# Minys233/GCN-BMP

Measured on AMD Instinct MI355X. Metric: drug-pairs/sec fwd+bwd, binary-DDI GGNN d=128, higher is better.
Workload: dtype f32; 1 GPU; C2: full binary DDI set (544 drugs, 147696 pairs), GGNN 4-step d=128 tied + Nie co-attention (head 8, tanh) + MLP(32,16), fwd+bwd+Adam, 1024 pairs/GPU/step, every molecule instance encoded; the 144 batches of one epoch resident in HBM, cycled; layout=per-instance packed layout, whole 128-row tiles, pairs_per_gpu=1024, global_batch=1024, parallelism=dp1

## Files before the change

gcn-bmp_amd/csrc/bmp_fused.hip:

```cpp
#include <type_traits>
#include <string.h>
#include "bmp_kernels.h"

#include "bmp_tile.h"

template <int D, bool FIRST, bool VAR, bool SAVE>
__global__ __launch_bounds__(512) void k_ggnn_step_fwd(StepArgs a) {
    constexpr int LD = D + 4;
    constexpr int NCB = D / 32, NRW = 8 / NCB, RB = 4 / NRW;
    extern __shared__ __attribute__((aligned(16))) float lds[];
    float* Hs = lds;
    float* As = lds + FZ_R * LD;
    float* wds = As + FZ_R * LD;
    int* rptr = (int*)(wds + FZ_R * 4);
    int* ecol = rptr + 132;
    float* evalv = (float*)(ecol + FZ_ECAP);
    int* sy = (int*)(evalv + FZ_ECAP);

    const int tid = threadIdx.x, lane = tid & 63, w = tid >> 6;
    const int grp = w >> 2;
    GrpSync gs{sy + grp, 0};
    if (tid < FZ_NSYNC) sy[tid] = 0;
    if (grp == 0) __builtin_amdgcn_s_setprio(2);
    const int wc = w % NCB, wr = w / NCB;
    const int l31 = lane & 31, hi = lane >> 5;
    FZ_TILE_SETUP();
    if (VAR && a.tile_stride > nrows) {
        const int e = row0 + a.tile_stride;
        fz_clear_rows<512>(a.hout, D, row0 + nrows, e, tid);
        fz_clear_rows<512>(a.m, D, row0 + nrows, e, tid);
        fz_clear_rows<512>(a.rz, 2 * D, row0 + nrows, e, tid);
        fz_clear_rows<512>(a.c, D, row0 + nrows, e, tid);
    }
    const int col = wc * 32 + l31;
    const int wrow0 = wr * RB * 32;
    const int lrow = wrow0 + 4 * hi;
    const int rot = (tile * 8) % D;
    const float* Hw = Hs + (wrow0 + l31) * LD + 4 * hi;
    const float* Aw = As + (wrow0 + l31) * LD + 4 * hi;
    float* Hl = Hs + lrow * LD + col;
    float* Al = As + lrow * LD + col;
#define LOFF(rb, reg) (((rb) * 32 + ((reg) & 3) + 8 * ((reg) >> 2)) * LD)

    constexpr bool save = SAVE;
    for (int idx = tid; idx < nrows * (D / 4); idx += 512) {
        const int r = idx / (D / 4), c4 = idx % (D / 4);
        *(f32x4*)(Hs + r * LD + 4 * c4) = *(const f32x4*)(a.h + (size_t)(row0 + r) * D + 4 * c4);
    }
    const bool csr_lds = stage_csr(a.ptr, a.col, a.val, row0, rptr, ecol, evalv, nrows);
    __syncthreads();
    if (!grp_live) return;
    const RowOrder ro = FZ_ROW_ORDER();
    const int bi = wr & 1;

    auto step = [&](auto first_c, const float* WTs, const float* bEs, const float* ATs, const float* bvs, float* om, float* orz,
                    float* oc, float* oh) {
        constexpr bool FST = decltype(first_c)::value;
        int tmask = 0;
        f32x16 acc_m[1][RB];
        zero_acc(acc_m[0]);
        for (int e = 0; e < 4; ++e) {
            const float* const Bp[1] = {WTs + (size_t)(e * D + 4 * hi) * D + 4 * col};
            const int ldw[1] = {D};
            BPre<1> pre;
            tile_b_prefetch<1>(pre, Bp, ldw, D, rot);
            float wd;
            FZ_GATHER(Hs, As, e, &wd);
            if ((tid & 3) == 0) wds[(tid >> 2) * 4 + e] = wd;
            if (e == 0 && (tid & 3) == 0 && tmask) __hip_atomic_fetch_or(sy + 2 + grp, tmask, __ATOMIC_RELAXED, __HIP_MEMORY_SCOPE_WORKGROUP);
            grp_sync(gs);
            const int any = (__hip_atomic_load(sy + 2 + grp, __ATOMIC_RELAXED, __HIP_MEMORY_SCOPE_WORKGROUP) >> e) & 1;
            if (any) tile_mma_msg<VAR, 1, RB>(nrb, e, ro.nbr, bi, acc_m, Aw, LD, Bp, ldw, D, rot, &pre);
            FZ_GSYNC();
        }
        constexpr int NG = FST ? 2 : 3;
        int ldwg[NG];
    #pragma unroll
        for (int g = 0; g < NG; ++g) ldwg[g] = 3 * D;
        const float* const base_h = ATs + (size_t)(4 * hi) * 3 * D + 4 * col + (FST ? 4 * D : 0);
        const float* const base_m = ATs + (size_t)(D + 4 * hi) * 3 * D + 4 * col + (FST ? 4 * D : 0);
        const float* Bh[NG]; const float* Bm[NG];
    #pragma unroll
        for (int g = 0; g < NG; ++g) { Bh[g] = base_h + 4 * D * g; Bm[g] = base_m + 4 * D * g; }
        BPre<NG> pre_h;
        tile_b_prefetch<NG>(pre_h, (const float* const (&)[NG])Bh, (const int (&)[NG])ldwg, D, rot);
        {
            const AccBuf mo = acc_buf<D>(om, row0, 0, col);
            float be[4];
    #pragma unroll
            for (int e = 0; e < 4; ++e) be[e] = bEs[e * D + col];
            FZ_FOR_ACC {
                const int tp = lrow + rb * 32 + (reg & 3) + 8 * (reg >> 2);
                const int r = (tp & 64) + ro.perm[tp];
                const f32x4 wd4 = *(const f32x4*)(wds + r * 4);
                const float v = __builtin_fmaf(wd4[3], be[3], __builtin_fmaf(wd4[2], be[2], __builtin_fmaf(wd4[1], be[1],
                                               __builtin_fmaf(wd4[0], be[0], acc_m[0][rb][reg]))));
                As[r * LD + col] = v;
                if (save) __builtin_amdgcn_raw_buffer_store_b32(__builtin_bit_cast(unsigned, v), mo.rs, mo.vo + r * D * 4, 0, 0);
            }
        }
        FZ_GSYNC();

        f32x16 acc_g[3][RB];
        zero_acc(acc_g[0]); zero_acc(acc_g[1]); zero_acc(acc_g[2]);
        {
            f32x16 gg[NG][RB];
    #pragma unroll
            for (int g = 0; g < NG; ++g) zero_acc(gg[g]);
            BPre<NG> pre_m;
            tile_b_prefetch<NG>(pre_m, (const float* const (&)[NG])Bm, (const int (&)[NG])ldwg, D, rot);
            tile_mma_n<VAR, NG, RB>(nrb, gg, Hw, LD, (const float* const (&)[NG])Bh, (const int (&)[NG])ldwg, D, rot, &pre_h);
            tile_mma_n<VAR, NG, RB>(nrb, gg, Aw, LD, (const float* const (&)[NG])Bm, (const int (&)[NG])ldwg, D, rot, &pre_m);
    #pragma unroll
            for (int g = 0; g < NG; ++g)
    #pragma unroll
                for (int rb = 0; rb < RB; ++rb) acc_g[g + (FST ? 1 : 0)][rb] = gg[g][rb];
        }
        const float br = bvs[col], bz = bvs[D + col], bcn = bvs[2 * D + col];
        {
            const AccBuf rzo = acc_buf<2 * D>(orz, row0, lrow, col);
            FZ_FOR_ACC {
                const float zv = bmp_sigmoid(acc_g[1][rb][reg] + bz);
                acc_g[1][rb][reg] = zv;
                if (save) acc_st<2 * D>(rzo, rb, reg, zv, D);
                if (!FST) {
                    const float rv = bmp_sigmoid(acc_g[0][rb][reg] + br);
                    acc_g[0][rb][reg] = rv;
                    if (save) acc_st<2 * D>(rzo, rb, reg, rv, 0);
                }
            }
        }
        if (!FST) {
            const float* const Bu[1] = {a.UcT + (size_t)(4 * hi) * D + 4 * col};
            const int ldu[1] = {D};
            BPre<1> pre_u;
            tile_b_prefetch<1>(pre_u, Bu, ldu, D, rot);
            FZ_GSYNC();
            FZ_FOR_ACC { Al[LOFF(rb, reg)] = acc_g[0][rb][reg] * Hl[LOFF(rb, reg)]; }
            FZ_GSYNC();
            f32x16 gc[1][RB];
    #pragma unroll
            for (int rb = 0; rb < RB; ++rb) gc[0][rb] = acc_g[2][rb];
            tile_mma_n<VAR, 1, RB>(nrb, gc, Aw, LD, Bu, ldu, D, rot, &pre_u);
    #pragma unroll
            for (int rb = 0; rb < RB; ++rb) acc_g[2][rb] = gc[0][rb];
        }
        {
            const AccBuf co = acc_buf<D>(oc, row0, lrow, col);
            const AccBuf ho = acc_buf<D>(oh, row0, lrow, col);
            FZ_FOR_ACC {
                const float cv = bmp_tanh(acc_g[2][rb][reg] + bcn);
                const float zv = acc_g[1][rb][reg];
                float hn = zv * cv;
                if (!FST) hn = __builtin_fmaf(1.f - zv, Hl[LOFF(rb, reg)], hn);
                if (save) acc_st<D>(co, rb, reg, cv);
                acc_st<D>(ho, rb, reg, hn);
            }
        }
    };
    step(std::integral_constant<bool, FIRST>{}, a.WT, a.bE, a.AT, a.b, a.m, a.rz, a.c, a.hout);
}

template <int D, bool FIRST, bool VAR>
__global__ __launch_bounds__(512) void k_ggnn_step_bwd(StepArgs a) {
    constexpr int LD = D + 4;
    constexpr int NCB = D / 32, NRW = 8 / NCB, RB = 4 / NRW;
    constexpr int F4 = D / 4;
    constexpr int NV = D / 16;
    extern __shared__ __attribute__((aligned(16))) float lds[];
    float* Xs = lds;
    float* Ys = lds + FZ_R * LD;
    int* rptr = (int*)(Ys + FZ_R * LD + FZ_R * 4);
    int* ecol = rptr + 132;
    float* evalv = (float*)(ecol + FZ_ECAP);
    int* sy = (int*)(evalv + FZ_ECAP);

    const int tid = threadIdx.x, lane = tid & 63, w = tid >> 6;
    const int grp = w >> 2;
    GrpSync gs{sy + grp, 0};
    int tmask = 0;
    if (tid < FZ_NSYNC) sy[tid] = 0;
    if (grp == 0) __builtin_amdgcn_s_setprio(2);
    const int wc = w % NCB, wr = w / NCB;
    const int l31 = lane & 31, hi = lane >> 5;
    FZ_TILE_SETUP();
    if (VAR && a.tile_stride > nrows) {
        const int e = row0 + a.tile_stride;
        fz_clear_rows<512>(a.dh, D, row0 + nrows, e, tid);
        fz_clear_rows<512>(a.gda, 7 * D, row0 + nrows, e, tid);
    }
    const int col = wc * 32 + l31;
    const int wrow0 = wr * RB * 32;
    const int lrow = wrow0 + 4 * hi;
    const int rot = (tile * 8) % D;
    const float* Xw = Xs + (wrow0 + l31) * LD + 4 * hi;
    const float* Yw = Ys + (wrow0 + l31) * LD + 4 * hi;
    float* Xl = Xs + lrow * LD + col;
    float* Yl = Ys + lrow * LD + col;
    constexpr bool first = FIRST;
    const int tg = tid & 255;
#define RM_ROW(v) (grp * 64 + ((v) * 256 + tg) / F4)
#define RM_C4(v) (((v) * 256 + tg) % F4)
#define RM_LDS(T, v) (*(f32x4*)((T) + RM_ROW(v) * LD + 4 * RM_C4(v)))
#define RM_LIVE(v) (!VAR || grp * 64 + (v) * (256 / F4) < nrows)
    const AccBuf b_g = rm_buf<D, D>(a.dhout, row0, grp, tg), b_c = rm_buf<D, D>(a.c, row0, grp, tg);
    const AccBuf b_h = rm_buf<D, D>(a.h, row0, grp, tg), b_rz = rm_buf<D, 2 * D>(a.rz, row0, grp, tg);
    const AccBuf b_o = rm_buf<D, 7 * D>(a.gda, row0, grp, tg), b_dh = rm_buf<D, D>(a.dh, row0, grp, tg);

    const bool csr_lds = stage_csr(a.ptr, a.col, a.val, row0, rptr, ecol, evalv, nrows);
    if (!grp_live) {
        __syncthreads();
        return;
    }

    f32x4 ex[NV];
    {
        const f32x4 one = (f32x4){1.f, 1.f, 1.f, 1.f};
        f32x4 g4[NV], z4[NV], c4[NV], h4[NV];
#pragma unroll
        for (int v = 0; v < NV; ++v) if (RM_LIVE(v)) {
            g4[v] = rm_ld<D, D>(b_g, v);
            z4[v] = rm_ld<D, 2 * D>(b_rz, v, D);
            c4[v] = rm_ld<D, D>(b_c, v);
            if (!first) h4[v] = rm_ld<D, D>(b_h, v);
        }
#pragma unroll
        for (int v = 0; v < NV; ++v) if (RM_LIVE(v)) {
            const f32x4 gz = g4[v] * z4[v];
            const f32x4 dac = gz * (one - c4[v] * c4[v]);
            f32x4 dz = gz * (one - z4[v]);
            if (first) { dz *= c4[v]; ex[v] = (f32x4){0.f, 0.f, 0.f, 0.f}; }
            else { dz *= (c4[v] - h4[v]); ex[v] = g4[v] - gz; }
            RM_LDS(Xs, v) = dac;
            RM_LDS(Ys, v) = dz;
            rm_st<D, 7 * D>(b_o, v, dac, 6 * D);
            rm_st<D, 7 * D>(b_o, v, dz, 5 * D);
        }
    }
    const float* const Ac_h = a.A + (size_t)(2 * D + 4 * hi) * 2 * D + 4 * col;
    const float* const Az_h = a.A + (size_t)(D + 4 * hi) * 2 * D + 4 * col;
    const float* const Ar_h = a.A + (size_t)(4 * hi) * 2 * D + 4 * col;
    const int ld2[2] = {2 * D, 2 * D};
    const float* const Bc[2] = {Ac_h, Ac_h + 4 * D};
    BPre<2> pre_c;
    tile_b_prefetch<2>(pre_c, Bc, ld2, D, rot);
    __syncthreads();
    const RowOrder ro = FZ_ROW_ORDER();
    const int bi = wr & 1;
    int aoff[RB];
#pragma unroll
    for (int rb = 0; rb < RB; ++rb) { const int tp = wrow0 + rb * 32 + l31; aoff[rb] = (((tp & 64) + ro.perm[tp]) - (wrow0 + l31)) * LD; }
#define FZ_ROWOF(rb, reg) ((lrow & 64) + ro.perm[lrow + (rb) * 32 + ((reg) & 3) + 8 * ((reg) >> 2)])

    f32x16 acc_x[2][RB];
    zero_acc(acc_x[0]); zero_acc(acc_x[1]);
    tile_mma_n<VAR, 2, RB>(nrb, acc_x, Xw, LD, Bc, ld2, D, rot, &pre_c, aoff);
    if (!first) {
        f32x16 acc_d[1][RB];
        zero_acc(acc_d[0]);
        {
            const float* const Bu[1] = {a.Uc + (size_t)(4 * hi) * D + 4 * col};
            const int ldu[1] = {D};
            tile_mma_n<VAR, 1, RB>(nrb, acc_d, Xw, LD, Bu, ldu, D, rot, nullptr, aoff);
        }
        FZ_GSYNC();
        FZ_FOR_ACC { Xs[FZ_ROWOF(rb, reg) * LD + col] = acc_d[0][rb][reg]; }
        f32x4 r4[NV], h4[NV];
#pragma unroll
        for (int v = 0; v < NV; ++v) if (RM_LIVE(v)) { r4[v] = rm_ld<D, 2 * D>(b_rz, v); h4[v] = rm_ld<D, D>(b_h, v); }
        FZ_GSYNC();
#pragma unroll
        for (int v = 0; v < NV; ++v) if (RM_LIVE(v)) {
            const f32x4 drh = RM_LDS(Xs, v);
            const f32x4 dr = drh * r4[v];
            const f32x4 dar = dr * h4[v] * ((f32x4){1.f, 1.f, 1.f, 1.f} - r4[v]);
            ex[v] += dr;
            RM_LDS(Xs, v) = dar;
            rm_st<D, 7 * D>(b_o, v, dar, 4 * D);
        }
        FZ_GSYNC();
        {
            const float* const Br[2] = {Ar_h, Ar_h + 4 * D};
            tile_mma_n<VAR, 2, RB>(nrb, acc_x, Xw, LD, Br, ld2, D, rot, nullptr, aoff);
        }
    }
    {
        const float* const Bz[2] = {Az_h, Az_h + 4 * D};
        tile_mma_n<VAR, 2, RB>(nrb, acc_x, Yw, LD, Bz, ld2, D, rot, nullptr, aoff);
    }
    FZ_GSYNC();
    FZ_FOR_ACC { Xs[FZ_ROWOF(rb, reg) * LD + col] = acc_x[1][rb][reg]; }
    __syncthreads();

    f32x16 acc_h[1][RB];
#pragma unroll
    for (int rb = 0; rb < RB; ++rb) acc_h[0][rb] = acc_x[0][rb];
    for (int e = 0; e < 4; ++e) {
        const float* const Bp[1] = {a.Wnat + (size_t)(4 * hi) * 4 * D + 4 * (e * D + col)};
        const int ldw[1] = {4 * D};
        BPre<1> pre;
        tile_b_prefetch<1>(pre, Bp, ldw, D, rot);
        float wd;
        const bool has_e = FZ_GATHER(Xs, Ys, e, &wd);
        if ((tid >> 2) < nrows && (has_e || !a.skip_zero_g)) {
            const int row = tid >> 2, q = tid & 3;
            const float* s = Ys + ((row & 64) + ro.inv[row]) * LD + q * (D / 4);
            float* o = a.gda + (size_t)(row0 + row) * 7 * D + e * D + q * (D / 4);
#pragma unroll
            for (int f = 0; f < D / 16; ++f) *(f32x4*)(o + 4 * f) = *(const f32x4*)(s + 4 * f);
        }
        if (e == 0 && (tid & 3) == 0 && tmask) __hip_atomic_fetch_or(sy + 2 + grp, tmask, __ATOMIC_RELAXED, __HIP_MEMORY_SCOPE_WORKGROUP);
        grp_sync(gs);
        const int any = (__hip_atomic_load(sy + 2 + grp, __ATOMIC_RELAXED, __HIP_MEMORY_SCOPE_WORKGROUP) >> e) & 1;
        if (any) tile_mma_msg<VAR, 1, RB>(nrb, e, ro.nbr, bi, acc_h, Yw, LD, Bp, ldw, D, rot, &pre);
        FZ_GSYNC();
    }
    FZ_FOR_ACC { Ys[FZ_ROWOF(rb, reg) * LD + col] = acc_h[0][rb][reg]; }
    FZ_GSYNC();
#pragma unroll
    for (int v = 0; v < NV; ++v) if (RM_LIVE(v)) rm_st<D, D>(b_dh, v, RM_LDS(Ys, v) + ex[v]);
#undef RM_LIVE
#undef RM_ROW
#undef RM_C4
#undef RM_LDS
#undef FZ_ROWOF
}

struct RelArgs {
    const int* ptr; const int* col; const float* val;
    int tile0;
    int act;
    const int* mt_row0; const int* mt_nblk;
    int mt_rows;
    const float* h;
    const float* WT;
    const float* bE;
    const float* WsT;
    const float* bs;
    float* out;
    float* wdeg;
    const float* dout; const float* y;
    const float* Wnat;
    const float* Ws;
    float* dh;
    float* gda;
    int skip_zero_g;
};

template <int D, bool VAR>
__global__ __launch_bounds__(512) void k_relgcn_layer_fwd(RelArgs a) {
    constexpr int LD = D + 4;
    constexpr int NCB = D / 32, NRW = 8 / NCB, RB = 4 / NRW;
    extern __shared__ __attribute__((aligned(16))) float lds[];
    float* Hs = lds;
    float* As = lds + FZ_R * LD;
    float* wds = As + FZ_R * LD;
    int* rptr = (int*)(wds + FZ_R * 4);
    int* ecol = rptr + 132;
    float* evalv = (float*)(ecol + FZ_ECAP);
    int* sy = (int*)(evalv + FZ_ECAP);

    const int tid = threadIdx.x, lane = tid & 63, w = tid >> 6;
    const int grp = w >> 2;
    GrpSync gs{sy + grp, 0};
    int tmask = 0;
    if (tid < FZ_NSYNC) sy[tid] = 0;
    if (grp == 0) __builtin_amdgcn_s_setprio(2);
    const int wc = w % NCB, wr = w / NCB;
    const int l31 = lane & 31, hi = lane >> 5;
    FZ_TILE_SETUP();
    const int col = wc * 32 + l31;
    const int wrow0 = wr * RB * 32;
    const int lrow = wrow0 + 4 * hi;
    const int rot = (tile * 8) % D;
    const float* Hw = Hs + (wrow0 + l31) * LD + 4 * hi;
    const float* Aw = As + (wrow0 + l31) * LD + 4 * hi;

    for (int idx = tid; idx < nrows * (D / 4); idx += 512) {
        const int r = idx / (D / 4), c4 = idx % (D / 4);
        *(f32x4*)(Hs + r * LD + 4 * c4) = *(const f32x4*)(a.h + (size_t)(row0 + r) * D + 4 * c4);
    }
    const bool csr_lds = stage_csr(a.ptr, a.col, a.val, row0, rptr, ecol, evalv, nrows);
    __syncthreads();
    if (!grp_live) return;
    const RowOrder ro = FZ_ROW_ORDER();
    const int bi = wr & 1;
    int aoff[RB];
#pragma unroll
    for (int rb = 0; rb < RB; ++rb) { const int tp = wrow0 + rb * 32 + l31; aoff[rb] = (((tp & 64) + ro.perm[tp]) - (wrow0 + l31)) * LD; }

    f32x16 acc[1][RB];
    zero_acc(acc[0]);
    const float* const Bs[1] = {a.WsT + (size_t)(4 * hi) * D + 4 * col};
    const int lds_[1] = {D};
    BPre<1> pre_s;
    for (int e = 0; e < 4; ++e) {
        const float* const Bp[1] = {a.WT + (size_t)(e * D + 4 * hi) * D + 4 * col};
        const int ldw[1] = {D};
        BPre<1> pre;
        tile_b_prefetch<1>(pre, Bp, ldw, D, rot);
        if (e == 3) tile_b_prefetch<1>(pre_s, Bs, lds_, D, rot);
        float wd;
        FZ_GATHER(Hs, As, e, &wd);
        if ((tid & 3) == 0) wds[(tid >> 2) * 4 + e] = wd;
        if (e == 0 && (tid & 3) == 0 && tmask) __hip_atomic_fetch_or(sy + 2 + grp, tmask, __ATOMIC_RELAXED, __HIP_MEMORY_SCOPE_WORKGROUP);
        grp_sync(gs);
        const int any = (__hip_atomic_load(sy + 2 + grp, __ATOMIC_RELAXED, __HIP_MEMORY_SCOPE_WORKGROUP) >> e) & 1;
        if (any) tile_mma_msg<VAR, 1, RB>(nrb, e, ro.nbr, bi, acc, Aw, LD, Bp, ldw, D, rot, &pre);
        FZ_GSYNC();
    }
    tile_mma_n<VAR, 1, RB>(nrb, acc, Hw, LD, Bs, lds_, D, rot, &pre_s, aoff);
    {
        const AccBuf oo = acc_buf<D>(a.out, row0, 0, col);
        float be[4];
#pragma unroll
        for (int e = 0; e < 4; ++e) be[e] = a.bE[e * D + col];
        const float bsv = a.bs ? a.bs[col] : 0.f;
        const int act = a.act;
        FZ_FOR_ACC {
            const int tp = lrow + rb * 32 + (reg & 3) + 8 * (reg >> 2);
            const int r = (tp & 64) + ro.perm[tp];
            const f32x4 wd4 = *(const f32x4*)(wds + r * 4);
            const float v = acc[0][rb][reg] + bsv + wd4[0] * be[0] + wd4[1] * be[1] + wd4[2] * be[2] + wd4[3] * be[3];
            __builtin_amdgcn_raw_buffer_store_b32(__builtin_bit_cast(unsigned, bmp_act(act, v)), oo.rs, oo.vo + r * D * 4, 0, 0);
        }
    }
    if (a.wdeg != nullptr && (tid & 255) < 64 && grp * 64 + (tid & 255) < nrows) {
        const int r = grp * 64 + (tid & 255);
        *(f32x4*)(a.wdeg + (size_t)(row0 + r) * 4) = *(const f32x4*)(wds + r * 4);
    }
}

template <int D, bool VAR>
__global__ __launch_bounds__(512) void k_relgcn_layer_bwd(RelArgs a) {
    constexpr int LD = D + 4;
    constexpr int NCB = D / 32, NRW = 8 / NCB, RB = 4 / NRW;
    constexpr int F4 = D / 4;
    constexpr int NV = D / 16;
    extern __shared__ __attribute__((aligned(16))) float lds[];
    float* Xs = lds;
    float* Ys = lds + FZ_R * LD;
    int* rptr = (int*)(Ys + FZ_R * LD + FZ_R * 4);
    int* ecol = rptr + 132;
    float* evalv = (float*)(ecol + FZ_ECAP);
    int* sy = (int*)(evalv + FZ_ECAP);

    const int tid = threadIdx.x, lane = tid & 63, w = tid >> 6;
    const int grp = w >> 2;
    GrpSync gs{sy + grp, 0};
    int tmask = 0;
    if (tid < FZ_NSYNC) sy[tid] = 0;
    if (grp == 0) __builtin_amdgcn_s_setprio(2);
    const int wc = w % NCB, wr = w / NCB;
    const int l31 = lane & 31, hi = lane >> 5;
    FZ_TILE_SETUP();
    const int col = wc * 32 + l31;
    const int wrow0 = wr * RB * 32;
    const int lrow = wrow0 + 4 * hi;
    const int rot = (tile * 8) % D;
    const float* Xw = Xs + (wrow0 + l31) * LD + 4 * hi;
    const float* Yw = Ys + (wrow0 + l31) * LD + 4 * hi;
    float* Yl = Ys + lrow * LD + col;
    const int tg = tid & 255;
#define RM_ROW(v) (grp * 64 + ((v) * 256 + tg) / F4)
#define RM_C4(v) (((v) * 256 + tg) % F4)
#define RM_LDS(T, v) (*(f32x4*)((T) + RM_ROW(v) * LD + 4 * RM_C4(v)))
#define RM_LIVE(v) (!VAR || grp * 64 + (v) * (256 / F4) < nrows)
    const AccBuf b_g = rm_buf<D, D>(a.dout, row0, grp, tg), b_y = rm_buf<D, D>(a.y, row0, grp, tg);
    const AccBuf b_o = rm_buf<D, 5 * D>(a.gda, row0, grp, tg), b_dh = rm_buf<D, D>(a.dh, row0, grp, tg);

    const bool csr_lds = stage_csr(a.ptr, a.col, a.val, row0, rptr, ecol, evalv, nrows);
    if (!grp_live) {
        __syncthreads();
        return;
    }

    {
        f32x4 g4[NV], y4[NV];
#pragma unroll
        for (int v = 0; v < NV; ++v) if (RM_LIVE(v)) { g4[v] = rm_ld<D, D>(b_g, v); y4[v] = rm_ld<D, D>(b_y, v); }
        const int act = a.act;
#pragma unroll
        for (int v = 0; v < NV; ++v) if (RM_LIVE(v)) {
            f32x4 dp;
#pragma unroll
            for (int t = 0; t < 4; ++t) dp[t] = g4[v][t] * bmp_dact(act, y4[v][t]);
            RM_LDS(Xs, v) = dp;
            rm_st<D, 5 * D>(b_o, v, dp, 4 * D);
        }
    }
    const float* const Bs[1] = {a.Ws + (size_t)(4 * hi) * D + 4 * col};
    const int lds_[1] = {D};
    BPre<1> pre_s;
    tile_b_prefetch<1>(pre_s, Bs, lds_, D, rot);
    __syncthreads();
    const RowOrder ro = FZ_ROW_ORDER();
    const int bi = wr & 1;
    int aoff[RB];
#pragma unroll
    for (int rb = 0; rb < RB; ++rb) { const int tp = wrow0 + rb * 32 + l31; aoff[rb] = (((tp & 64) + ro.perm[tp]) - (wrow0 + l31)) * LD; }

    f32x16 acc_h[1][RB];
    zero_acc(acc_h[0]);
    tile_mma_n<VAR, 1, RB>(nrb, acc_h, Xw, LD, Bs, lds_, D, rot, &pre_s, aoff);
    for (int e = 0; e < 4; ++e) {
        const float* const Bp[1] = {a.Wnat + (size_t)(4 * hi) * 4 * D + 4 * (e * D + col)};
        const int ldw[1] = {4 * D};
        BPre<1> pre;
        tile_b_prefetch<1>(pre, Bp, ldw, D, rot);
        float wd;
        const bool has_e = FZ_GATHER(Xs, Ys, e, &wd);
        if ((tid >> 2) < nrows && (has_e || !a.skip_zero_g)) {
            const int row = tid >> 2, q = tid & 3;
            const float* s = Ys + ((row & 64) + ro.inv[row]) * LD + q * (D / 4);
            float* o = a.gda + (size_t)(row0 + row) * 5 * D + e * D + q * (D / 4);
#pragma unroll
            for (int f = 0; f < D / 16; ++f) *(f32x4*)(o + 4 * f) = *(const f32x4*)(s + 4 * f);
        }
        if (e == 0 && (tid & 3) == 0 && tmask) __hip_atomic_fetch_or(sy + 2 + grp, tmask, __ATOMIC_RELAXED, __HIP_MEMORY_SCOPE_WORKGROUP);
        grp_sync(gs);
        const int any = (__hip_atomic_load(sy + 2 + grp, __ATOMIC_RELAXED, __HIP_MEMORY_SCOPE_WORKGROUP) >> e) & 1;
        if (any) tile_mma_msg<VAR, 1, RB>(nrb, e, ro.nbr, bi, acc_h, Yw, LD, Bp, ldw, D, rot, &pre);
        FZ_GSYNC();
    }
    FZ_FOR_ACC {
        const int tp = lrow + rb * 32 + (reg & 3) + 8 * (reg >> 2);
        Ys[((tp & 64) + ro.perm[tp]) * LD + col] = acc_h[0][rb][reg];
    }
    FZ_GSYNC();
#pragma unroll
    for (int v = 0; v < NV; ++v) if (RM_LIVE(v)) rm_st<D, D>(b_dh, v, RM_LDS(Ys, v));
#undef RM_LIVE
#undef RM_ROW
#undef RM_C4
#undef RM_LDS
}

struct ROArgs {
    const float* h; const float* h0;
    const float* WT;
    const float* b;
    int act_j;
    const float* row_w; const int* row_mol; const int* mol_nrows;
    float* ij;
    float* g;
};

template <int D, bool HAS0>
__global__ __launch_bounds__(512) void k_readout_tile_fwd(ROArgs a) {
    constexpr int LD = D + 4;
    constexpr int NCB = D / 32, NRW = 8 / NCB, RB = 4 / NRW;
    extern __shared__ __attribute__((aligned(16))) float lds[];
    float* Hs = lds;
    float* As = lds + FZ_R * LD;
    int* mlist = (int*)(As + FZ_R * LD);
    float* rws = (float*)(mlist + 400);
    const int tid = threadIdx.x, lane = tid & 63, w = tid >> 6;
    const int wc = w % NCB, wr = w / NCB;
    const int l31 = lane & 31, hi = lane >> 5;
    const int row0 = blockIdx.x * FZ_R;
    const int col = wc * 32 + l31;
    const int wrow0 = wr * RB * 32;
    const int lrow = wrow0 + 4 * hi;
    const int rot = (blockIdx.x * 8) % D;
    constexpr int nrb = RB;
    const float* Hw = Hs + (wrow0 + l31) * LD + 4 * hi;
    const float* Aw = As + (wrow0 + l31) * LD + 4 * hi;
    float* Al = As + lrow * LD + col;

    for (int idx = tid; idx < FZ_R * (D / 4); idx += 512) {
        const int r = idx / (D / 4), c4 = idx % (D / 4);
        *(f32x4*)(Hs + r * LD + 4 * c4) = *(const f32x4*)(a.h + (size_t)(row0 + r) * D + 4 * c4);
        if (HAS0) *(f32x4*)(As + r * LD + 4 * c4) = *(const f32x4*)(a.h0 + (size_t)(row0 + r) * D + 4 * c4);
    }
    if (tid < FZ_R) rws[tid] = a.row_w[row0 + tid];
    const float* const Bh[2] = {a.WT + (size_t)(4 * hi) * 2 * D + 4 * col, a.WT + (size_t)(4 * hi) * 2 * D + 4 * (D + col)};
    const int ldw[2] = {2 * D, 2 * D};
    BPre<2> pre_h;
    tile_b_prefetch<2>(pre_h, Bh, ldw, D, rot);
    __syncthreads();

    f32x16 acc[2][RB];
    zero_acc(acc[0]); zero_acc(acc[1]);
    if (HAS0) {
        const float* const B0[2] = {Bh[0] + (size_t)D * 2 * D, Bh[1] + (size_t)D * 2 * D};
        BPre<2> pre_0;
        tile_b_prefetch<2>(pre_0, B0, ldw, D, rot);
        tile_mma<2, RB>(acc, Hw, LD, Bh, ldw, D, rot, &pre_h);
        tile_mma<2, RB>(acc, Aw, LD, B0, ldw, D, rot, &pre_0);
    } else {
        tile_mma<2, RB>(acc, Hw, LD, Bh, ldw, D, rot, &pre_h);
    }
    if (tid < FZ_R) {
        const int mol = a.row_mol[row0 + tid];
        const int prev = tid > 0 ? a.row_mol[row0 + tid - 1] : -2;
        const bool head = mol >= 0 && mol != prev;
        const unsigned long long bal = __ballot(head);
        if (lane == 0) mlist[128 + w] = __popcll(bal);
        const int before = __popcll(bal & ((1ull << lane) - 1ull));
        if (head) { mlist[130 + tid] = before; }
        mlist[260 + tid] = head ? mol : -1;
    }
    __syncthreads();
    {
        const AccBuf io = acc_buf<2 * D>(a.ij, row0, lrow, col);
        const float bi = a.b ? a.b[col] : 0.f, bj = a.b ? a.b[D + col] : 0.f;
        const int act = a.act_j;
        FZ_FOR_ACC {
            const int r = lrow + rb * 32 + (reg & 3) + 8 * (reg >> 2);
            const float iv = bmp_sigmoid(acc[0][rb][reg] + bi);
            const float jv = bmp_act(act, acc[1][rb][reg] + bj);
            if (a.ij != nullptr) {
                acc_st<2 * D>(io, rb, reg, iv, 0);
                acc_st<2 * D>(io, rb, reg, jv, D);
            }
            Al[LOFF(rb, reg)] = rws[r] * iv * jv;
        }
    }
    if (tid < FZ_R && mlist[260 + tid] >= 0) {
        const int idx = mlist[130 + tid] + (tid >= 64 ? mlist[128] : 0);
        mlist[2 * idx] = tid;
        mlist[2 * idx + 1] = mlist[260 + tid];
    }
// ... 255 lines not shown
```

gcn-bmp_amd/csrc/bmp_tile.h:

```cpp
#pragma once
#include <stdlib.h>
#include <type_traits>
#include <string.h>
#include "bmp_kernels.h"

#define FZ_R 128

struct StepArgs {
    const int* ptr; const int* col; const float* val;
    int tile0;
    int first;
    const int* mt_row0; const int* mt_nblk;
    int mt_rows;
    const float* h;
    const float* WT;
    const float* bE;
    const float* AT;
    const float* UcT;
    const float* b;
    float* m; float* rz; float* c; float* hout;
    const float* dhout;
    const float* Wnat;
    const float* A;
    const float* Uc;
    float* dh;
    float* gda;
    int skip_zero_g;
    int tile_stride;
};

template <int NT>
__device__ __forceinline__ void fz_clear_rows(float* p, int W, int r_begin, int r_end, int tid) {
    if (p == nullptr) return;
    const int w4 = W >> 2;
    f32x4* q = (f32x4*)(p + (size_t)r_begin * W);
    const int n = (r_end - r_begin) * w4;
    for (int i = tid; i < n; i += NT) q[i] = (f32x4){0.f, 0.f, 0.f, 0.f};
}

template <int NB>
struct BPre { f32x4 b0[NB], b1[NB]; };
template <int NB>
__device__ __forceinline__ void tile_b_prefetch(BPre<NB>& p, const float* const (&Bp)[NB], const int (&ldw)[NB], int K, int rot) {
    int k1 = rot + 8; if (k1 >= K) k1 -= K;
#pragma unroll
    for (int nb = 0; nb < NB; ++nb) {
        p.b0[nb] = *(const f32x4*)(Bp[nb] + (size_t)rot * ldw[nb]);
        p.b1[nb] = *(const f32x4*)(Bp[nb] + (size_t)k1 * ldw[nb]);
    }
}

template <int NB, int RB, int NRB = RB>
__device__ __forceinline__ void tile_mma(f32x16 (&acc)[NB][RB], const float* As_wave, int LD, const float* const (&Bp)[NB],
                                         const int (&ldw)[NB], int K, int rot, const BPre<NB>* pre = nullptr, const int* aoff = nullptr) {
    f32x4 b0[NB], b1[NB], b2[NB];
    int k = rot;
    int k1 = k + 8; if (k1 >= K) k1 -= K;
#pragma unroll
    for (int nb = 0; nb < NB; ++nb) {
        if (pre) { b0[nb] = pre->b0[nb]; b1[nb] = pre->b1[nb]; }
        else {
            b0[nb] = *(const f32x4*)(Bp[nb] + (size_t)k * ldw[nb]);
            b1[nb] = *(const f32x4*)(Bp[nb] + (size_t)k1 * ldw[nb]);
        }
    }
    f32x4 a0[NRB], a1[NRB];
#pragma unroll
    for (int rb = 0; rb < NRB; ++rb) a0[rb] = *(const f32x4*)(As_wave + (aoff ? aoff[rb] : rb * 32 * LD) + k);
    for (int it = 0; it < K; it += 8) {
        int k2 = k1 + 8; if (k2 >= K) k2 -= K;
#pragma unroll
        for (int nb = 0; nb < NB; ++nb) b2[nb] = *(const f32x4*)(Bp[nb] + (size_t)k2 * ldw[nb]);
#pragma unroll
        for (int rb = 0; rb < NRB; ++rb) a1[rb] = *(const f32x4*)(As_wave + (aoff ? aoff[rb] : rb * 32 * LD) + k1);
        __builtin_amdgcn_sched_barrier(0);
#pragma unroll
        for (int t = 0; t < 4; ++t)
#pragma unroll
            for (int rb = 0; rb < NRB; ++rb)
#pragma unroll
                for (int nb = 0; nb < NB; ++nb) acc[nb][rb] = bmp_mfma(a0[rb][t], b0[nb][t], acc[nb][rb]);
        __builtin_amdgcn_sched_barrier(0);
#pragma unroll
        for (int nb = 0; nb < NB; ++nb) { b0[nb] = b1[nb]; b1[nb] = b2[nb]; }
#pragma unroll
        for (int rb = 0; rb < NRB; ++rb) a0[rb] = a1[rb];
        k = k1; k1 = k2;
    }
}

template <bool VAR, int NB, int RB>
__device__ __forceinline__ void tile_mma_n(int nrb, f32x16 (&acc)[NB][RB], const float* As_wave, int LD, const float* const (&Bp)[NB],
                                           const int (&ldw)[NB], int K, int rot, const BPre<NB>* pre = nullptr, const int* aoff = nullptr) {
    if constexpr (!VAR) {
        tile_mma<NB, RB, RB>(acc, As_wave, LD, Bp, ldw, K, rot, pre, aoff);
    } else if constexpr (RB == 1) {
        if (nrb > 0) tile_mma<NB, 1, 1>(acc, As_wave, LD, Bp, ldw, K, rot, pre, aoff);
    } else {
        if (nrb == RB) tile_mma<NB, RB, RB>(acc, As_wave, LD, Bp, ldw, K, rot, pre, aoff);
        else if (nrb > 0) tile_mma<NB, RB, 1>(acc, As_wave, LD, Bp, ldw, K, rot, pre, aoff);
    }
}

template <int N>
__device__ __forceinline__ void zero_acc(f32x16 (&acc)[N]) {
#pragma unroll
    for (int i = 0; i < N; ++i)
#pragma unroll
        for (int r = 0; r < 16; ++r) acc[i][r] = 0.f;
}

template <int D>
__device__ __forceinline__ bool tile_gather(const float* src_tile, float* dst_tile, int LD, const int* ptr, const int* col,
                                            const float* val, int row0, int e, float* wsum, int* tmask, int nrows = FZ_R,
                                            const unsigned char* inv = nullptr) {
    constexpr int F = D / 16;
    const int row = threadIdx.x >> 2, q = threadIdx.x & 3;
    f32x4 acc[F];
#pragma unroll
    for (int f = 0; f < F; ++f) acc[f] = (f32x4){0.f, 0.f, 0.f, 0.f};
    float wd = 0.f;
    bool any = false;
    *wsum = 0.f;
    if (nrows < FZ_R && row >= nrows) return false;
    const int e0 = ptr[row], e1 = ptr[row + 1];
    for (int ed = e0; ed < e1; ++ed) {
        const int cv = col[ed];
        *tmask |= 1 << (cv & 3);
        if ((cv & 3) == e) {
            const float v = val[ed];
            const float* s = src_tile + ((cv >> 2) - row0) * LD + q * (D / 4);
#pragma unroll
            for (int f = 0; f < F; ++f) acc[f] += *(const f32x4*)(s + 4 * f) * v;
            wd += v;
            any = true;
        }
    }
    float* o = dst_tile + (inv ? (row & 64) + inv[row] : row) * LD + q * (D / 4);
#pragma unroll
    for (int f = 0; f < F; ++f) *(f32x4*)(o + 4 * f) = acc[f];
    *wsum = wd;
    return any;
}

#define FZ_ECAP 1024
__device__ __forceinline__ bool stage_csr(const int* ptr, const int* col, const float* val, int row0, int* rptr, int* ecol,
                                          float* evalv, int nrows = FZ_R, int nt = 512) {
    const int ebase = ptr[row0];
    const int ne = ptr[row0 + nrows] - ebase;
    if (ne > FZ_ECAP) return false;
    for (int i = threadIdx.x; i <= nrows; i += nt) rptr[i] = ptr[row0 + i] - ebase;
    for (int i = threadIdx.x; i < ne; i += nt) { ecol[i] = col[ebase + i]; evalv[i] = val[ebase + i]; }
    return true;
}
#define FZ_GATHER(srcT, dstT, e, wdp) (csr_lds ? tile_gather<D>(srcT, dstT, LD, rptr, ecol, evalv, row0, e, wdp, &tmask, nrows, ro.inv) \
                                               : tile_gather<D>(srcT, dstT, LD, a.ptr + row0, a.col, a.val, row0, e, wdp, &tmask, nrows, ro.inv))
#define FZ_ROW_ORDER() fz_row_order(sy, gs, grp, w, lane, csr_lds ? rptr : a.ptr + row0, csr_lds ? ecol : a.col, nrows)

struct GrpSync {
    int* ctr;
    int target;
};
__device__ __forceinline__ void grp_sync(GrpSync& g) {
    g.target += 4;
    __builtin_amdgcn_fence(__ATOMIC_RELEASE, "workgroup", "local");
    if ((threadIdx.x & 63) == 0) __hip_atomic_fetch_add(g.ctr, 1, __ATOMIC_RELAXED, __HIP_MEMORY_SCOPE_WORKGROUP);
    while (__hip_atomic_load(g.ctr, __ATOMIC_RELAXED, __HIP_MEMORY_SCOPE_WORKGROUP) < g.target) __builtin_amdgcn_s_sleep(1);
    __builtin_amdgcn_fence(__ATOMIC_ACQUIRE, "workgroup", "local");
}
#define FZ_NSYNC 72

#define FZ_RARE_TYPES 0x6
struct RowOrder {
    const unsigned char* inv;
    const unsigned char* perm;
    int nbr;
};
__device__ __forceinline__ RowOrder fz_row_order(int* sy, GrpSync& gs, int grp, int w, int lane, const int* ptr_local, const int* col,
                                                 int nrows) {
    unsigned char* inv = (unsigned char*)(sy + 8);
    unsigned char* perm = (unsigned char*)(sy + 40);
    if ((w & 3) == 0) {
        const int r = grp * 64 + lane;
        int m = 0;
        if (r < nrows)
            for (int ed = ptr_local[r]; ed < ptr_local[r + 1]; ++ed) m |= 1 << (col[ed] & 3);
        const bool rare = (m & FZ_RARE_TYPES) != 0;
        const unsigned long long bal = __ballot(rare), lt = (1ull << lane) - 1ull;
        const int nr = __popcll(bal);
        const int pos = rare ? __popcll(bal & lt) : nr + __popcll(~bal & lt);
        inv[r] = (unsigned char)pos;
        perm[grp * 64 + pos] = (unsigned char)lane;
        if (lane == 0) sy[4 + grp] = nr;
    }
    grp_sync(gs);
    return RowOrder{inv, perm, (sy[4 + grp] + 31) >> 5};
}
template <bool VAR, int NB, int RB>
__device__ __forceinline__ void tile_mma_msg(int nrb, int e, int nbr, int bi, f32x16 (&acc)[NB][RB], const float* As_wave, int LD,
                                             const float* const (&Bp)[NB], const int (&ldw)[NB], int K, int rot, const BPre<NB>* pre) {
    const bool rare = (FZ_RARE_TYPES >> e) & 1;
    if constexpr (RB == 1) {
        if (nrb > 0 && (!rare || bi < nbr)) tile_mma<NB, 1, 1>(acc, As_wave, LD, Bp, ldw, K, rot, pre);
    } else {
        const int nb = rare ? (nbr < nrb ? nbr : nrb) : nrb;
        if (nb >= RB) tile_mma<NB, RB, RB>(acc, As_wave, LD, Bp, ldw, K, rot, pre);
        else if (nb > 0) tile_mma<NB, RB, 1>(acc, As_wave, LD, Bp, ldw, K, rot, pre);
    }
}

struct AccBuf {
    __amdgpu_buffer_rsrc_t rs;
    int vo;
};
template <int LDC>
__device__ __forceinline__ AccBuf acc_buf(const float* base, int tile_row0, int lane_row, int col) {
    AccBuf b;
    b.rs = __builtin_amdgcn_make_buffer_rsrc((void*)(base + (size_t)tile_row0 * LDC), 0, 0x7FFFFFFF, 0x00020000);
    b.vo = (lane_row * LDC + col) * 4;
    return b;
}
template <int LDC>
__device__ __forceinline__ float acc_ld(const AccBuf& b, int rb, int reg, int coff = 0) {
    const int so = ((rb * 32 + (reg & 3) + 8 * (reg >> 2)) * LDC + coff) * 4;
    return __builtin_bit_cast(float, __builtin_amdgcn_raw_buffer_load_b32(b.rs, b.vo, so, 0));
}
template <int LDC>
__device__ __forceinline__ void acc_st(const AccBuf& b, int rb, int reg, float v, int coff = 0) {
    const int so = ((rb * 32 + (reg & 3) + 8 * (reg >> 2)) * LDC + coff) * 4;
    __builtin_amdgcn_raw_buffer_store_b32(__builtin_bit_cast(unsigned, v), b.rs, b.vo, so, 0);
}

typedef unsigned u32x4 __attribute__((ext_vector_type(4)));
template <int D, int LDP>
__device__ __forceinline__ AccBuf rm_buf(const float* base, int tile_row0, int grp, int tg) {
    AccBuf b;
    b.rs = __builtin_amdgcn_make_buffer_rsrc((void*)(base + (size_t)tile_row0 * LDP), 0, 0x7FFFFFFF, 0x00020000);
    b.vo = ((grp * 64 + tg / (D / 4)) * LDP + 4 * (tg % (D / 4))) * 4;
    return b;
}
template <int D, int LDP>
__device__ __forceinline__ f32x4 rm_ld(const AccBuf& b, int v, int coff = 0) {
    const int so = (v * (1024 / D) * LDP + coff) * 4;
    return __builtin_bit_cast(f32x4, __builtin_amdgcn_raw_buffer_load_b128(b.rs, b.vo, so, 0));
}
template <int D, int LDP>
__device__ __forceinline__ void rm_st(const AccBuf& b, int v, f32x4 x, int coff = 0) {
    const int so = (v * (1024 / D) * LDP + coff) * 4;
    __builtin_amdgcn_raw_buffer_store_b128(__builtin_bit_cast(u32x4, x), b.rs, b.vo + so, 0, 0);
}

#define FZ_FOR_ACC _Pragma("unroll") for (int rb = 0; rb < RB; ++rb) if (rb < nrb) _Pragma("unroll") for (int reg = 0; reg < 16; ++reg)

template <int D>
__device__ __forceinline__ int fz_live(int nblk, int wr) {
    constexpr int NCB = D / 32, NRW = 8 / NCB, RB = 4 / NRW;
    const int live = nblk - wr * RB;
    return live < 0 ? 0 : (live > RB ? RB : live);
}
#define FZ_TILE_SETUP()                                                          \
    const int tile = blockIdx.x + a.tile0;                                      \
    const int row0 = VAR ? a.mt_row0[tile] : tile * FZ_R;                       \
    const int nblk = VAR ? a.mt_nblk[tile] : 4;                                 \
    const int nrows = VAR ? nblk * 32 : FZ_R;                                   \
    const int nrb = VAR ? fz_live<D>(nblk, wr) : RB;                            \
    const bool grp_live = VAR ? nblk > 2 * grp : true

#define FZ_GSYNC() grp_sync(gs)
```

Measured before the change: 402,900 pairs/s.

## Prefetch all GGNN backward B-tiles early and spill residual gradient to HBM

In the GGNN step backward kernel, B-operand prefetches for the Uc, Ar and Az weight tiles are issued ahead of their MMAs instead of only for Ac. The residual gradient ex is stored to the dh buffer mid-kernel and reloaded at the end, so it no longer occupies registers through the four-edge message loop. The r/h loads are reordered to overlap with the MMA, and an opaque-asm wrapper on rot stops the compiler from hoisting or merging address arithmetic. This trades extra global traffic and more prefetch registers for lower register pressure and better latency hiding.

```diff
diff --git a/gcn-bmp_amd/csrc/bmp_fused.hip b/gcn-bmp_amd/csrc/bmp_fused.hip
--- a/gcn-bmp_amd/csrc/bmp_fused.hip
+++ b/gcn-bmp_amd/csrc/bmp_fused.hip
@@ -161,6 +161,16 @@
     step(std::integral_constant<bool, FIRST>{}, a.WT, a.bE, a.AT, a.b, a.m, a.rz, a.c, a.hout);
 }
 
+template <bool FUSE>
+__device__ __forceinline__ f32x4 fz_mul_add(f32x4 a, f32x4 b, f32x4 c) {
+    if constexpr (FUSE) return __builtin_elementwise_fma(a, b, c);
+    else {
+#pragma clang fp contract(off)
+        const f32x4 p = a * b;
+        return p + c;
+    }
+}
+
 template <int D, bool FIRST, bool VAR>
 __global__ __launch_bounds__(512) void k_ggnn_step_bwd(StepArgs a) {
     constexpr int LD = D + 4;
@@ -229,7 +239,7 @@
             const f32x4 gz = g4[v] * z4[v];
             const f32x4 dac = gz * (one - c4[v] * c4[v]);
             f32x4 dz = gz * (one - z4[v]);
-            if (first) { dz *= c4[v]; ex[v] = (f32x4){0.f, 0.f, 0.f, 0.f}; }
+            if (first) dz *= c4[v];
             else { dz *= (c4[v] - h4[v]); ex[v] = g4[v] - gz; }
             RM_LDS(Xs, v) = dac;
             RM_LDS(Ys, v) = dz;
@@ -242,8 +252,15 @@
     const float* const Ar_h = a.A + (size_t)(4 * hi) * 2 * D + 4 * col;
     const int ld2[2] = {2 * D, 2 * D};
     const float* const Bc[2] = {Ac_h, Ac_h + 4 * D};
-    BPre<2> pre_c;
+    const float* const Bz[2] = {Az_h, Az_h + 4 * D};
+    const float* const Br[2] = {Ar_h, Ar_h + 4 * D};
+    const float* const Bu[1] = {a.Uc + (size_t)(4 * hi) * D + 4 * col};
+    const int ldu[1] = {D};
+    BPre<2> pre_c, pre_r, pre_z;
+    BPre<1> pre_u;
     tile_b_prefetch<2>(pre_c, Bc, ld2, D, rot);
+    if (first) tile_b_prefetch<2>(pre_z, Bz, ld2, D, rot);
+    else tile_b_prefetch<1>(pre_u, Bu, ldu, D, rot);
     __syncthreads();
     const RowOrder ro = FZ_ROW_ORDER();
     const int bi = wr & 1;
@@ -254,40 +271,34 @@
 
     f32x16 acc_x[2][RB];
     zero_acc(acc_x[0]); zero_acc(acc_x[1]);
-    tile_mma_n<VAR, 2, RB>(nrb, acc_x, Xw, LD, Bc, ld2, D, rot, &pre_c, aoff);
+    tile_mma_n<VAR, 2, RB>(nrb, acc_x, Xw, LD, Bc, ld2, D, fz_opaque(rot), &pre_c, aoff);
     if (!first) {
         f32x16 acc_d[1][RB];
         zero_acc(acc_d[0]);
-        {
-            const float* const Bu[1] = {a.Uc + (size_t)(4 * hi) * D + 4 * col};
-            const int ldu[1] = {D};
-            tile_mma_n<VAR, 1, RB>(nrb, acc_d, Xw, LD, Bu, ldu, D, rot, nullptr, aoff);
-        }
+        f32x4 r4[NV], h4[NV];
+#pragma unroll
+        for (int v = 0; v < NV; ++v) if (RM_LIVE(v)) r4[v] = rm_ld<D, 2 * D>(b_rz, v);
+        tile_mma_n<VAR, 1, RB>(nrb, acc_d, Xw, LD, Bu, ldu, D, fz_opaque(rot), &pre_u, aoff);
         FZ_GSYNC();
         FZ_FOR_ACC { Xs[FZ_ROWOF(rb, reg) * LD + col] = acc_d[0][rb][reg]; }
-        f32x4 r4[NV], h4[NV];
-#pragma unroll
-        for (int v = 0; v < NV; ++v) if (RM_LIVE(v)) { r4[v] = rm_ld<D, 2 * D>(b_rz, v); h4[v] = rm_ld<D, D>(b_h, v); }
+#pragma unroll
+        for (int v = 0; v < NV; ++v) if (RM_LIVE(v)) h4[v] = rm_ld<D, D>(b_h, v);
+        tile_b_prefetch<2>(pre_r, Br, ld2, D, rot);
         FZ_GSYNC();
 #pragma unroll
         for (int v = 0; v < NV; ++v) if (RM_LIVE(v)) {
             const f32x4 drh = RM_LDS(Xs, v);
             const f32x4 dr = drh * r4[v];
             const f32x4 dar = dr * h4[v] * ((f32x4){1.f, 1.f, 1.f, 1.f} - r4[v]);
-            ex[v] += dr;
+            ex[v] = fz_mul_add<VAR>(drh, r4[v], ex[v]);
             RM_LDS(Xs, v) = dar;
             rm_st<D, 7 * D>(b_o, v, dar, 4 * D);
+            rm_st<D, D>(b_dh, v, ex[v]);
         }
         FZ_GSYNC();
-        {
-            const float* const Br[2] = {Ar_h, Ar_h + 4 * D};
-            tile_mma_n<VAR, 2, RB>(nrb, acc_x, Xw, LD, Br, ld2, D, rot, nullptr, aoff);
-        }
-    }
-    {
-        const float* const Bz[2] = {Az_h, Az_h + 4 * D};
-        tile_mma_n<VAR, 2, RB>(nrb, acc_x, Yw, LD, Bz, ld2, D, rot, nullptr, aoff);
-    }
+        tile_mma_n<VAR, 2, RB>(nrb, acc_x, Xw, LD, Br, ld2, D, fz_opaque(rot), &pre_r, aoff);
+    }
+    tile_mma_n<VAR, 2, RB>(nrb, acc_x, Yw, LD, Bz, ld2, D, fz_opaque(rot), first ? &pre_z : nullptr, aoff);
     FZ_GSYNC();
     FZ_FOR_ACC { Xs[FZ_ROWOF(rb, reg) * LD + col] = acc_x[1][rb][reg]; }
     __syncthreads();
@@ -315,10 +326,18 @@
         if (any) tile_mma_msg<VAR, 1, RB>(nrb, e, ro.nbr, bi, acc_h, Yw, LD, Bp, ldw, D, rot, &pre);
         FZ_GSYNC();
     }
+    f32x4 pk[NV];
+    if (!first) {
+#pragma unroll
+        for (int v = 0; v < NV; ++v) if (RM_LIVE(v)) pk[v] = rm_ld<D, D>(b_dh, v);
+    }
     FZ_FOR_ACC { Ys[FZ_ROWOF(rb, reg) * LD + col] = acc_h[0][rb][reg]; }
     FZ_GSYNC();
 #pragma unroll
-    for (int v = 0; v < NV; ++v) if (RM_LIVE(v)) rm_st<D, D>(b_dh, v, RM_LDS(Ys, v) + ex[v]);
+    for (int v = 0; v < NV; ++v) if (RM_LIVE(v)) {
+        if (first) rm_st<D, D>(b_dh, v, RM_LDS(Ys, v));
+        else rm_st<D, D>(b_dh, v, RM_LDS(Ys, v) + pk[v]);
+    }
 #undef RM_LIVE
 #undef RM_ROW
 #undef RM_C4
diff --git a/gcn-bmp_amd/csrc/bmp_tile.h b/gcn-bmp_amd/csrc/bmp_tile.h
--- a/gcn-bmp_amd/csrc/bmp_tile.h
+++ b/gcn-bmp_amd/csrc/bmp_tile.h
@@ -102,6 +102,8 @@
     }
 }
 
+__device__ __forceinline__ int fz_opaque(int x) { asm volatile("" : "+s"(x)); return x; }
+
 template <int N>
 __device__ __forceinline__ void zero_acc(f32x16 (&acc)[N]) {
 #pragma unroll
```

Result: faster. 407,000 pairs/s, median of 6 (+1.0%).
